# WangFeng18/3d-gaussian-splatting

Hardware: NVIDIA H100
Metric: render+backward FPS @1080p (2.4M Gaussians) (higher is better)
Workload: dtype f32

## Files before the change

### 3d-gaussian-splatting_b200/csrc/internal.h

```cpp
#pragma once
#include <cuda_runtime.h>
#include <stdint.h>

#include "../../include/gs_b200.h"
#include "project.cuh"

#define GS_GREC 12

struct GsFrameGeom {
  int width, height, wp, hp, ntx, nty, n_tiles;
  float fx, fy;
};

struct GsCrop {
  int left, top, width, height;
};

struct GsAuxOut {
  float bg[3];
  float* aux;
  float* aux_final;
};

#ifdef __CUDACC__
__device__ __forceinline__ void gs_store_aux(const GsAuxOut& ax, int ix, int iy, int wp, const GsCrop& crop,
                                             float depth, float alpha) {
  if (ax.aux) *reinterpret_cast<float2*>(ax.aux + ((size_t)iy * wp + ix) * 2) = make_float2(depth, alpha);
  const int x = ix - crop.left, y = iy - crop.top;
  if (ax.aux_final && x >= 0 && x < crop.width && y >= 0 && y < crop.height)
    *reinterpret_cast<float2*>(ax.aux_final + ((size_t)y * crop.width + x) * 2) = make_float2(depth, alpha);
}
template <int PX>
__device__ __forceinline__ void gs_load_aux_grad(const float* __restrict__ aux, const float* __restrict__ grad_aux,
                                                 int grad_is_final, int ix0, int iy, int wp, const GsCrop& crop,
                                                 float (&gD)[PX], float (&gA)[PX], float (&R)[PX]) {
#pragma unroll
  for (int p = 0; p < PX; ++p) {
    const size_t off = ((size_t)iy * wp + ix0 + p) * 2;
    const float2 da = *reinterpret_cast<const float2*>(aux + off);
    float2 g = make_float2(0.f, 0.f);
    if (!grad_is_final) {
      g = *reinterpret_cast<const float2*>(grad_aux + off);
    } else {
      const int x = ix0 + p - crop.left, y = iy - crop.top;
      if (x >= 0 && x < crop.width && y >= 0 && y < crop.height)
        g = *reinterpret_cast<const float2*>(grad_aux + ((size_t)y * crop.width + x) * 2);
    }
    gD[p] = g.x;
    gA[p] = g.y;
    R[p] = fmaf(g.x, da.x, fmaf(g.y, da.y, R[p]));
  }
}
#endif

struct GsRayPtrs {
  const float *rays_o, *lefttop, *dx, *dy;
};

struct GsTuning {
  int fwd_kernel;
  int fwd_ch;
  int bwd_kernel;
  int bwd_px;
  int bwd_ws;
  int bwd_unroll;
  int bwd_stages;
  int bwd_minb;
  int bwd_rq;
  int fwd_px;
  int bwd_ch;
  int strict;
  int gather;
  int sh_tc;
  int blend_repack;
};
GsTuning& gs_tuning();

void gs_count_launch(int n = 1);

int gs_sh_basis_count(int d);
int gs_sh_stream_width(int d);
int gs_sh_grad_width(int d);
int gs_sh_tc_mode(int d);
cudaError_t gs_launch_blend_sh_fwd(const float4* pA, const float2* pB, const float* pS, const GsRec* grec,
                                   const float* rgb, const uint32_t* ids, const uint32_t* goff , int d,
                                   const int* tile_accum,
                                   const GsFrameGeom& g, const GsRayPtrs& r, float* image, int* tile_neff,
                                   float* final_img, const GsCrop& crop, cudaStream_t st,
                                   const GsAuxOut* aux = nullptr );
cudaError_t gs_launch_blend_sh_bwd(const float4* pA, const float2* pB, const float* pS, const GsRec* grec,
                                   const float* rgb, const uint32_t* ids, const uint32_t* goff , int d,
                                   const int* tile_accum,
                                   const GsFrameGeom& g, const GsRayPtrs& r, const float* image,
                                   const float* grad_image, float* grad_inst, int grad_is_final, const GsCrop& crop,
                                   uint32_t* row_epoch, uint32_t epoch, int* tile_neff_b, cudaStream_t st,
                                   const float* aux = nullptr, const float* grad_aux = nullptr );

cudaError_t gs_launch_blend_sh_fwd_tc(const GsRec* grec, const float* rgb, const uint32_t* ids, int d,
                                      const int* tile_accum, const GsFrameGeom& g, const GsRayPtrs& r, float* image,
                                      int* tile_neff, float* final_img, const GsCrop& crop, cudaStream_t st,
                                      const GsAuxOut* aux = nullptr);
cudaError_t gs_launch_blend_sh_bwd_tc(const GsRec* grec, const float* rgb, const uint32_t* ids, const uint32_t* goff, int d,
                                      const int* tile_accum, const GsFrameGeom& g, const GsRayPtrs& r, const float* image,
                                      const float* grad_image, float* grad_inst, int grad_is_final, const GsCrop& crop,
                                      uint32_t* row_epoch, uint32_t epoch, int* tile_neff_b, cudaStream_t st,
                                      const float* aux = nullptr, const float* grad_aux = nullptr);

cudaError_t gs_launch_fused_project(const float* pos, const float* rgb, const float* opa, const float* quat,
                                    const float* scale, int n, int d, int scale_act, const GsCam& cam,
                                    const GsTileGrid& grid, float near_plane, float half_w, float half_h,
                                    GsRec* rec, uint2* rect ,
                                    uint32_t* count, uint32_t* dkey, int64_t* mask, unsigned int* n_visible, cudaStream_t st,
                                    bool sh_gaussian = false ,
                                    const GsFilter2d* filt = nullptr ,
                                    const float* f3d = nullptr ,
                                    const GsLens* lens = nullptr );

struct GsView {
  GsCam cam;
  GsTileGrid grid;
  GsFilter2d filt;
  float half_w, half_h, fx, fy;
};

cudaError_t gs_launch_fused_project_batch(const float* pos, const float* rgb, const float* opa, const float* quat,
                                          const float* scale, int n, int n_views, int d, int scale_act,
                                          const GsView* views, float near_plane, GsRec* rec ,
                                          uint2* rect , uint32_t* count , uint32_t* dkey ,
                                          int64_t* mask , unsigned int* n_visible,
                                          cudaStream_t st, bool sh_gaussian, bool filt,
                                          const float* f3d = nullptr ,
                                          const GsLens* lenses = nullptr );

struct GsGradPush {
  float* bucket;
// ... 167 lines not shown
```

### 3d-gaussian-splatting_b200/csrc/project.cu

```cuda
#include "internal.h"
#include "sh_common.cuh"

namespace {

constexpr int kBlock = 256;
constexpr float kInf = __builtin_huge_valf();

__global__ void __launch_bounds__(kBlock) jacobian_kernel(const float* __restrict__ pc, int n,
                                                           float* __restrict__ jac) {
  int i = blockIdx.x * kBlock + threadIdx.x;
  if (i >= n) return;
  float u0 = pc[3 * i], u1 = pc[3 * i + 1], u2 = pc[3 * i + 2];
  float rs = rsqrtf(u0 * u0 + u1 * u1 + u2 * u2);
  float* j = jac + 9 * (size_t)i;
  j[0] = 1.f / u2;
  j[1] = 0.f;
  j[2] = -u0 / (u2 * u2);
  j[3] = 0.f;
  j[4] = 1.f / u2;
  j[5] = -u1 / (u2 * u2);
  j[6] = rs * u0;
  j[7] = rs * u1;
  j[8] = rs * u2;
}


__device__ __forceinline__ void view_dir(const GsCam& cam, const float p[3], float dir[3], float& inv_len) {
  float u[3];
#pragma unroll
  for (int j = 0; j < 3; ++j) u[j] = p[j] + (cam.r[j] * cam.t[0] + cam.r[3 + j] * cam.t[1] + cam.r[6 + j] * cam.t[2]);
  inv_len = 1.f / sqrtf(u[0] * u[0] + u[1] * u[1] + u[2] * u[2]);
#pragma unroll
  for (int j = 0; j < 3; ++j) dir[j] = u[j] * inv_len;
}

template <int K>
__device__ __forceinline__ void sh_logits(const float* coef, const float* Y, float l[3]) {
#pragma unroll
  for (int c = 0; c < 3; ++c) {
    float s = 0.f;
#pragma unroll
    for (int k = 0; k < K; ++k) s = fmaf(Y[k], coef[c * K + k], s);
    l[c] = s;
  }
}

template <int KG, bool F = false, bool G3 = false, bool L = false>
__device__ __forceinline__ void fused_project_body(
    const float* __restrict__ pos, const float* __restrict__ rgb, const float* __restrict__ opa,
    const float* __restrict__ quat, const float* __restrict__ scale, int n, int d, int scale_act, const GsCam& cam,
    const GsTileGrid& grid, float near_plane, float half_w, float half_h, GsRec* __restrict__ rec,
    uint2* __restrict__ rect, uint32_t* __restrict__ count, uint32_t* __restrict__ dkey, int64_t* __restrict__ mask,
    unsigned int* __restrict__ n_visible, GsFilter2d filt = GsFilter2d{}, const float* __restrict__ f3d = nullptr,
    GsLens lens = GsLens{}) {
  static_assert(!G3 || F, "the 3-D filter runs in the 2-D filter's kernels");
  static_assert(!L || G3, "the lens runs in the 3-D filter's kernels");
  int i = blockIdx.x * kBlock + threadIdx.x;
  bool vis = false;
  uint32_t cnt = 0;
  if (i < n) {
    float p[3] = {pos[3 * i], pos[3 * i + 1], pos[3 * i + 2]};
    float q[4], s[3], raw_s[3], qn;
    gs_load_activated(quat, scale, i, scale_act, q, s, raw_s, qn);
    float f3 = 0.f, dl2o3 = 0.f;
    if constexpr (G3) {
      float s0[3];
      f3 = (L && !f3d) ? 0.f : f3d[i];
      gs_filter3d(f3, s, s0, dl2o3);
    }
    const float opa_raw = opa[i];
    float rgb_raw[3] = {0.f, 0.f, 0.f};
    if (KG == 0 && d == 3) {
      rgb_raw[0] = rgb[3 * i];
      rgb_raw[1] = rgb[3 * i + 1];
      rgb_raw[2] = rgb[3 * i + 2];
    }
    GsProj o = gs_project(cam, p, q, s, near_plane, L ? kInf : half_w, L ? kInf : half_h);
    if constexpr (L) {
      float J[4];
      gs_lens_project(lens, o, half_w, half_h, J);
    }
    vis = o.visible;
    if (mask) mask[i] = o.visible ? 1 : 0;
    bool keep = o.visible;
    float dl2o = 0.f;
    if constexpr (F) {
      const GsFilter2dOut fo = gs_filter2d(filt, o.a, o.b, o.c, o.d);
      o.a = fo.a;
      o.d = fo.d;
      dl2o = fo.dl2o;
      keep = keep && fo.keep;
    }
    uint2 rc = make_uint2(0u, 0u);
    if (keep) {
      uint32_t tx0, tx1, ty0, ty1;
      if (gs_tile_rect(grid, o.x, o.y, o.a, o.b, o.c, o.d, tx0, tx1, ty0, ty1)) {
        cnt = (tx1 - tx0) * (ty1 - ty0);
        rc = make_uint2(tx0 | (ty0 << 16), (tx1 - tx0) | ((ty1 - ty0) << 16));
        GsConic k = gs_make_conic(o.a, o.b, o.c, o.d);
        float op = gs_sigmoid(opa_raw);
        GsRec* r = rec + i;
        r->a = make_float4(o.x, o.y, k.ca, k.cb);
        float cr = 0.f, cg = 0.f, cb = 0.f;
        if constexpr (KG > 0) {
          float coef[3 * KG], dir[3], il, Y[KG], l[3];
#pragma unroll
          for (int k = 0; k < 3 * KG; ++k) coef[k] = rgb[(size_t)i * (3 * KG) + k];
          view_dir(cam, p, dir, il);
          gs_sh::sh_basis<KG>(dir[0], dir[1], dir[2], Y);
          sh_logits<KG>(coef, Y, l);
          cr = gs_sigmoid(l[0]);
          cg = gs_sigmoid(l[1]);
          cb = gs_sigmoid(l[2]);
        } else if (d == 3) {
          cr = gs_sigmoid(rgb_raw[0]);
          cg = gs_sigmoid(rgb_raw[1]);
          cb = gs_sigmoid(rgb_raw[2]);
        }
        float l2o = log2f(op);
        if constexpr (G3) {
          if (f3 != 0.f) l2o += dl2o3;
        }
        r->b = make_float4(k.cc, F ? l2o + dl2o : l2o, cr, cg);
        r->c = make_float4(cb, o.depth, __uint_as_float(rc.x), __uint_as_float(rc.y));
        r->d = make_uint4(0u, 0u, 0u, 0u);
      }
    }
    rect[i] = rc;
    count[i] = cnt;
    dkey[i] = cnt ? __float_as_uint(o.depth) : 0xffffffffu;
  }
  __shared__ unsigned long long wsum[kBlock / 32];
  unsigned long long c64 = cnt;
#pragma unroll
  for (int o = 16; o; o >>= 1) c64 += __shfl_xor_sync(0xffffffffu, c64, o);
  if ((threadIdx.x & 31) == 0) wsum[threadIdx.x >> 5] = c64;
  int nv = __syncthreads_count(vis);
  if (threadIdx.x == 0) {
    unsigned long long tot = 0;
#pragma unroll
    for (int w = 0; w < kBlock / 32; ++w) tot += wsum[w];
    if (nv) atomicAdd(n_visible, (unsigned int)nv);
    if (tot) atomicAdd(reinterpret_cast<unsigned long long*>(n_visible + 2), tot);
  }
}

__global__ void __launch_bounds__(kBlock) fused_project_kernel(
    const float* __restrict__ pos, const float* __restrict__ rgb, const float* __restrict__ opa,
    const float* __restrict__ quat, const float* __restrict__ scale, int n, int d, int scale_act, GsCam cam,
    GsTileGrid grid, float near_plane, float half_w, float half_h, GsRec* __restrict__ rec,
    uint2* __restrict__ rect, uint32_t* __restrict__ count, uint32_t* __restrict__ dkey, int64_t* __restrict__ mask,
    unsigned int* __restrict__ n_visible) {
  fused_project_body<0>(pos, rgb, opa, quat, scale, n, d, scale_act, cam, grid, near_plane, half_w, half_h, rec, rect,
                        count, dkey, mask, n_visible);
}

template <int K>
__global__ void __launch_bounds__(kBlock) fused_project_sh_kernel(
    const float* __restrict__ pos, const float* __restrict__ rgb, const float* __restrict__ opa,
    const float* __restrict__ quat, const float* __restrict__ scale, int n, int scale_act, GsCam cam,
    GsTileGrid grid, float near_plane, float half_w, float half_h, GsRec* __restrict__ rec,
    uint2* __restrict__ rect, uint32_t* __restrict__ count, uint32_t* __restrict__ dkey, int64_t* __restrict__ mask,
    unsigned int* __restrict__ n_visible) {
  fused_project_body<K>(pos, rgb, opa, quat, scale, n, 3 * K, scale_act, cam, grid, near_plane, half_w, half_h, rec,
                        rect, count, dkey, mask, n_visible);
}

template <int K>
__global__ void __launch_bounds__(kBlock) fused_project_filt_kernel(
    const float* __restrict__ pos, const float* __restrict__ rgb, const float* __restrict__ opa,
    const float* __restrict__ quat, const float* __restrict__ scale, int n, int d, int scale_act, GsCam cam,
    GsTileGrid grid, float near_plane, float half_w, float half_h, GsRec* __restrict__ rec,
    uint2* __restrict__ rect, uint32_t* __restrict__ count, uint32_t* __restrict__ dkey, int64_t* __restrict__ mask,
    unsigned int* __restrict__ n_visible, GsFilter2d filt) {
  fused_project_body<K, true>(pos, rgb, opa, quat, scale, n, d, scale_act, cam, grid, near_plane, half_w, half_h, rec,
                              rect, count, dkey, mask, n_visible, filt);
}

template <int K>
__global__ void __launch_bounds__(kBlock) fused_project_filt3_kernel(
    const float* __restrict__ pos, const float* __restrict__ rgb, const float* __restrict__ opa,
    const float* __restrict__ quat, const float* __restrict__ scale, int n, int d, int scale_act, GsCam cam,
    GsTileGrid grid, float near_plane, float half_w, float half_h, GsRec* __restrict__ rec,
    uint2* __restrict__ rect, uint32_t* __restrict__ count, uint32_t* __restrict__ dkey, int64_t* __restrict__ mask,
    unsigned int* __restrict__ n_visible, GsFilter2d filt, const float* __restrict__ f3d) {
  fused_project_body<K, true, true>(pos, rgb, opa, quat, scale, n, d, scale_act, cam, grid, near_plane, half_w, half_h,
                                    rec, rect, count, dkey, mask, n_visible, filt, f3d);
}

template <int K>
__global__ void __launch_bounds__(kBlock) fused_project_lens_kernel(
    const float* __restrict__ pos, const float* __restrict__ rgb, const float* __restrict__ opa,
    const float* __restrict__ quat, const float* __restrict__ scale, int n, int d, int scale_act, GsCam cam,
    GsTileGrid grid, float near_plane, float half_w, float half_h, GsRec* __restrict__ rec,
    uint2* __restrict__ rect, uint32_t* __restrict__ count, uint32_t* __restrict__ dkey, int64_t* __restrict__ mask,
    unsigned int* __restrict__ n_visible, GsFilter2d filt, const float* __restrict__ f3d, GsLens lens) {
  fused_project_body<K, true, true, true>(pos, rgb, opa, quat, scale, n, d, scale_act, cam, grid, near_plane, half_w,
                                          half_h, rec, rect, count, dkey, mask, n_visible, filt, f3d, lens);
}

template <int KG, bool F, bool G3 = false, bool L = false>
__device__ __forceinline__ uint32_t fused_project_one(
    const float* __restrict__ rgb, int i, int d, const GsCam& cam, const GsTileGrid& grid, float near_plane,
    float half_w, float half_h, const GsFilter2d& filt, const float p[3], const float q[4], const float s[3],
    float opa_raw, const float rgb_raw[3], uint32_t ty_off, int j, GsRec* __restrict__ rec, uint2* __restrict__ rect,
    uint32_t* __restrict__ count, uint32_t* __restrict__ dkey, int64_t* __restrict__ mask, bool& vis,
    float f3 = 0.f, float dl2o3 = 0.f, const GsLens* __restrict__ lens = nullptr) {
  uint32_t cnt = 0;
  {
    GsProj o = gs_project(cam, p, q, s, near_plane, L ? kInf : half_w, L ? kInf : half_h);
    if constexpr (L) {
      float J[4];
      gs_lens_project(*lens, o, half_w, half_h, J);
    }
    vis = o.visible;
    if (mask) mask[j] = o.visible ? 1 : 0;
    bool keep = o.visible;
    float dl2o = 0.f;
    if constexpr (F) {
      const GsFilter2dOut fo = gs_filter2d(filt, o.a, o.b, o.c, o.d);
      o.a = fo.a;
      o.d = fo.d;
      dl2o = fo.dl2o;
      keep = keep && fo.keep;
    }
    uint2 rc = make_uint2(0u, 0u);
    if (keep) {
      uint32_t tx0, tx1, ty0, ty1;
      if (gs_tile_rect(grid, o.x, o.y, o.a, o.b, o.c, o.d, tx0, tx1, ty0, ty1)) {
        cnt = (tx1 - tx0) * (ty1 - ty0);
        rc = make_uint2(tx0 | ((ty0 + ty_off) << 16), (tx1 - tx0) | ((ty1 - ty0) << 16));
        GsConic k = gs_make_conic(o.a, o.b, o.c, o.d);
        float op = gs_sigmoid(opa_raw);
        GsRec* r = rec + j;
        r->a = make_float4(o.x, o.y, k.ca, k.cb);
        float cr = 0.f, cg = 0.f, cb = 0.f;
        if constexpr (KG > 0) {
          float coef[3 * KG], dir[3], il, Y[KG], l[3];
#pragma unroll
          for (int k = 0; k < 3 * KG; ++k) coef[k] = rgb[(size_t)i * (3 * KG) + k];
          view_dir(cam, p, dir, il);
          gs_sh::sh_basis<KG>(dir[0], dir[1], dir[2], Y);
          sh_logits<KG>(coef, Y, l);
          cr = gs_sigmoid(l[0]);
          cg = gs_sigmoid(l[1]);
          cb = gs_sigmoid(l[2]);
        } else if (d == 3) {
          cr = gs_sigmoid(rgb_raw[0]);
          cg = gs_sigmoid(rgb_raw[1]);
          cb = gs_sigmoid(rgb_raw[2]);
        }
        float l2o = log2f(op);
        if constexpr (G3) {
          if (f3 != 0.f) l2o += dl2o3;
        }
        r->b = make_float4(k.cc, F ? l2o + dl2o : l2o, cr, cg);
        r->c = make_float4(cb, o.depth, __uint_as_float(rc.x), __uint_as_float(rc.y));
        r->d = make_uint4(0u, 0u, 0u, 0u);
      }
    }
    rect[j] = rc;
    count[j] = cnt;
    dkey[j] = cnt ? __float_as_uint(o.depth) : 0xffffffffu;
  }
  return cnt;
}

template <int K, bool F, bool G3, bool L = false>
__device__ __forceinline__ void fused_project_batch_body(
    const float* __restrict__ pos, const float* __restrict__ rgb, const float* __restrict__ opa,
    const float* __restrict__ quat, const float* __restrict__ scale, int n, int n_views, int d, int scale_act,
    const GsView* __restrict__ views, float near_plane, GsRec* __restrict__ rec, uint2* __restrict__ rect,
    uint32_t* __restrict__ count, uint32_t* __restrict__ dkey, int64_t* __restrict__ mask,
    unsigned int* __restrict__ n_visible, const float* __restrict__ f3d, const GsLens* __restrict__ lenses = nullptr) {
  const int i = blockIdx.x * kBlock + threadIdx.x;
  unsigned int nv = 0;
  unsigned long long c64 = 0;
  if (i < n) {
    float p[3] = {pos[3 * i], pos[3 * i + 1], pos[3 * i + 2]};
    float q[4], s[3], raw_s[3], qn;
    gs_load_activated(quat, scale, i, scale_act, q, s, raw_s, qn);
    float f3 = 0.f, dl2o3 = 0.f;
    if constexpr (G3) {
      float s0[3];
      f3 = (L && !f3d) ? 0.f : f3d[i];
      gs_filter3d(f3, s, s0, dl2o3);
    }
    const float opa_raw = opa[i];
    float rgb_raw[3] = {0.f, 0.f, 0.f};
    if (K == 0 && d == 3) {
      rgb_raw[0] = rgb[3 * i];
      rgb_raw[1] = rgb[3 * i + 1];
      rgb_raw[2] = rgb[3 * i + 2];
    }
    for (int v = 0; v < n_views; ++v) {
      const GsView vw = views[v];
      bool vis = false;
      c64 += fused_project_one<K, F, G3, L>(rgb, i, d, vw.cam, vw.grid, near_plane, vw.half_w, vw.half_h, vw.filt, p,
                                            q, s, opa_raw, rgb_raw, (uint32_t)(v * vw.grid.nty), v * n + i, rec, rect,
                                            count, dkey, mask, vis, f3, dl2o3, lenses + v);
      nv += vis ? 1u : 0u;
    }
  }
  __shared__ unsigned long long wsum[kBlock / 32];
  __shared__ unsigned int wvis[kBlock / 32];
#pragma unroll
  for (int o = 16; o; o >>= 1) {
    c64 += __shfl_xor_sync(0xffffffffu, c64, o);
    nv += __shfl_xor_sync(0xffffffffu, nv, o);
  }
  if ((threadIdx.x & 31) == 0) {
    wsum[threadIdx.x >> 5] = c64;
    wvis[threadIdx.x >> 5] = nv;
  }
  __syncthreads();
  if (threadIdx.x == 0) {
    unsigned long long tot = 0;
    unsigned int tv = 0;
#pragma unroll
    for (int w = 0; w < kBlock / 32; ++w) {
      tot += wsum[w];
      tv += wvis[w];
    }
    if (tv) atomicAdd(n_visible, tv);
    if (tot) atomicAdd(reinterpret_cast<unsigned long long*>(n_visible + 2), tot);
  }
}

#define GS_PBATCH_PARAMS                                                                                            \
  const float* __restrict__ pos, const float* __restrict__ rgb, const float* __restrict__ opa,                     \
      const float* __restrict__ quat, const float* __restrict__ scale, int n, int n_views, int d, int scale_act,   \
      const GsView* __restrict__ views, float near_plane, GsRec* __restrict__ rec, uint2* __restrict__ rect,        \
      uint32_t* __restrict__ count, uint32_t* __restrict__ dkey, int64_t* __restrict__ mask,                        \
      unsigned int* __restrict__ n_visible
#define GS_PBATCH_ARGS \
  pos, rgb, opa, quat, scale, n, n_views, d, scale_act, views, near_plane, rec, rect, count, dkey, mask, n_visible

template <int K, bool F>
__global__ void __launch_bounds__(kBlock) fused_project_batch_kernel(GS_PBATCH_PARAMS) {
  fused_project_batch_body<K, F, false>(GS_PBATCH_ARGS, nullptr);
}

template <int K>
__global__ void __launch_bounds__(kBlock) fused_project_batch_filt3_kernel(GS_PBATCH_PARAMS,
                                                                           const float* __restrict__ f3d) {
  fused_project_batch_body<K, true, true>(GS_PBATCH_ARGS, f3d);
}

template <int K>
__global__ void __launch_bounds__(kBlock) fused_project_batch_lens_kernel(GS_PBATCH_PARAMS,
                                                                          const float* __restrict__ f3d,
                                                                          const GsLens* __restrict__ lenses) {
  fused_project_batch_body<K, true, true, true>(GS_PBATCH_ARGS, f3d, lenses);
}
#undef GS_PBATCH_PARAMS

template <int W>
__device__ __forceinline__ float* push_dst(const GsGradPush& P, float* local, int cnt) {
  if (W == 0) return local;
  const uint32_t idx = (uint32_t)(local - P.bucket);
  const uint32_t owner = idx / P.per;
  if (cnt > 1 && (idx + (uint32_t)cnt - 1) / P.per != owner) return nullptr;
  if (owner == (uint32_t)P.rank) return local;
  float* st = P.staging[0];
#pragma unroll
  for (int p = 1; p < (W > 0 ? W : 1); ++p)
    if (owner == (uint32_t)p) st = P.staging[p];
  return st + (size_t)P.rank * P.per + (idx - owner * P.per);
}

template <int W, int CNT>
__device__ __forceinline__ void push_store(const GsGradPush& P, float* local, const float* v) {
  float* dst = push_dst<W>(P, local, CNT);
  if (dst) {
#pragma unroll
    for (int k = 0; k < CNT; ++k) dst[k] = v[k];
  } else {
#pragma unroll
    for (int k = 0; k < CNT; ++k) *push_dst<W>(P, local + k, 1) = v[k];
  }
}

template <int D, int GW, int W, bool DT, int KG, bool CG = false, bool F = false, bool G3 = false, bool L = false>
__device__ __forceinline__ void fused_project_bwd_body(
    const float* __restrict__ pos, const float* __restrict__ rgb, const float* __restrict__ opa,
    const float* __restrict__ quat, const float* __restrict__ scale, int n, int scale_act, GsCam cam,
    float near_plane, float half_w, float half_h, const uint32_t* __restrict__ offsets_g,
    const uint32_t* __restrict__ count, const float* __restrict__ grad_inst,
    const uint32_t* __restrict__ row_epoch, uint32_t epoch, float* __restrict__ g_pos,
    float* __restrict__ g_rgb, float* __restrict__ g_opa, float* __restrict__ g_quat, float* __restrict__ g_scale,
    GsGradPush push, float* cg = nullptr, GsFilter2d filt = GsFilter2d{}, const float* __restrict__ f3d = nullptr,
    GsLens lens = GsLens{}) {
  static_assert(KG == 0 || (D == 3 * KG && GW == GS_GREC), "per-Gaussian SH: 3K coefficients, RGB gradient rows");
  static_assert(!G3 || F, "the 3-D filter runs in the 2-D filter's kernels");
  static_assert(!L || (G3 && W == 0), "the lens runs in the 3-D filter's kernels, without a push");
  static_assert(!CG || (W == 0 && GW == GS_GREC), "camera gradient: RGB gradient rows, no push");
  constexpr int DC = KG ? 3 : D;
  int i = blockIdx.x * kBlock + threadIdx.x;
  constexpr bool kStagedRgb = (D != 3) && (W == 0);
  const bool valid = i < n;
  if (!valid && !kStagedRgb) return;
  float gp[3] = {0.f, 0.f, 0.f}, gq_raw[4] = {0.f, 0.f, 0.f, 0.f}, gs_raw[3] = {0.f, 0.f, 0.f};
  float go = 0.f;
  float acc[GW];
#pragma unroll
  for (int k = 0; k < GW; ++k) acc[k] = 0.f;
  float gsh[KG ? D : 1];
#pragma unroll
// ... 1204 lines not shown
```

### 3d-gaussian-splatting_b200/csrc/render.cu

```cuda
#include <cub/device/device_radix_sort.cuh>
#include <cub/device/device_scan.cuh>
#include <cub/iterator/counting_input_iterator.cuh>
#include <cub/iterator/transform_input_iterator.cuh>

#include <cmath>
#include <cstdio>
#include <cstdlib>
#include <cstring>
#include <new>

#include "internal.h"

struct GsCountInSortedOrder {
  const uint32_t* count;
  const uint32_t* perm;
  uint32_t n;
  __host__ __device__ __forceinline__ uint32_t operator()(uint32_t i) const { return i < n ? count[perm[i]] : 0u; }
};

static thread_local char g_err[512] = {0};

int gs_set_error(cudaError_t e, const char* what) {
  snprintf(g_err, sizeof(g_err), "CUDA error %d (%s) at %s", (int)e, cudaGetErrorString(e), what);
  return (int)e;
// ... 340 lines not shown
    const double c[5] = {1.0, 3.0 * l.k[0], 5.0 * l.k[1], 7.0 * l.k[2], 9.0 * l.k[3]};
    const double half_pi = 1.5707963267948966;
    const double t = first_nonpositive(c, 4, half_pi * half_pi);
    if (!(t < half_pi * half_pi)) return INFINITY;
    const double r = tan(sqrt(t));
    return r * r;
  }
  return INFINITY;
}

static bool lens_is_centre_pinhole(const gs_lens& l, const gs_camera& cam) {
  return l.model == GS_LENS_PINHOLE && (double)l.cx == cam.width / 2.0 && (double)l.cy == cam.height / 2.0;
}

static GsLens lens_constants(const gs_lens& l, const gs_camera& cam) {
  GsLens L{};
  L.model = l.model;
  L.ox = (float)(((double)l.cx - cam.width / 2.0) / (double)cam.focal_x);
  L.oy = (float)(((double)l.cy - cam.height / 2.0) / (double)cam.focal_y);
  L.rho2_max = (float)lens_rho2_max(l);
  if (l.model != GS_LENS_PINHOLE)
    for (int k = 0; k < 4; ++k) L.k[k] = l.k[k];
  return L;
}

static int resolve_lenses(const gs_ctx* c, const gs_camera* cams, int n_views, GsLens* out, bool& on, const char* who) {
  on = false;
  if (c->lens_n == 0) return 0;
  if (c->lens_n != 1 && c->lens_n != n_views)
    return gs_fail(GS_ERR_INVALID_ARG, who, "the context's lenses are set for another number of views (n must be 1 or B)");
  for (int v = 0; v < n_views; ++v) {
    const gs_lens& l = c->lens_set[c->lens_n == 1 ? 0 : v];
    if (!lens_is_centre_pinhole(l, cams[v])) on = true;
    out[v] = lens_constants(l, cams[v]);
  }
  return 0;
}

static GsView view_constants(const gs_ctx* c, const gs_camera* cam, const GsFrameGeom& g) {
  GsView v{};
  if (c->filter2d != GS_FILTER2D_NONE) {
    v.filt.ex = (float)((double)c->filter2d_var / ((double)cam->focal_x * (double)cam->focal_x));
    v.filt.ey = (float)((double)c->filter2d_var / ((double)cam->focal_y * (double)cam->focal_y));
    v.filt.compensate = c->filter2d == GS_FILTER2D_ANTIALIAS;
  }
  v.grid.lx = (float)(16.0 / (double)cam->focal_x);
  v.grid.ly = (float)(16.0 / (double)cam->focal_y);
  v.grid.leftmost = (float)(-(double)g.wp / 2.0 / (double)cam->focal_x);
  v.grid.topmost = (float)(-(double)g.hp / 2.0 / (double)cam->focal_y);
  v.grid.t2 = -2.f * logf(cam->tile_thresh);
  v.grid.ntx = g.wp / GS_TILE;
  v.grid.nty = g.hp / GS_TILE;
  memcpy(v.cam.r, cam->rot, sizeof(v.cam.r));
  memcpy(v.cam.t, cam->tran, sizeof(v.cam.t));
  v.half_w = (float)((double)cam->width * 1.2 / 2.0 / (double)cam->focal_x);
  v.half_h = (float)((double)cam->height * 1.2 / 2.0 / (double)cam->focal_y);
  v.fx = cam->focal_x;
  v.fy = cam->focal_y;
  return v;
}

static int reserve_frame(gs_ctx* c, size_t N, int n_tiles, cudaStream_t st) {
  GS_CUDA_TRY(c->rec.reserve(N * sizeof(GsRec), st));
  GS_CUDA_TRY(c->rect.reserve(N * sizeof(uint2), st));
  GS_CUDA_TRY(c->count.reserve((N + 1) * 4, st));
  GS_CUDA_TRY(c->offsets.reserve((N + 1) * 4, st));
  GS_CUDA_TRY(c->dkey_in.reserve(N * 4 + 4, st));
  GS_CUDA_TRY(c->dkey_out.reserve(N * 4 + 4, st));
  GS_CUDA_TRY(c->perm.reserve(N * 4 + 4, st));
  GS_CUDA_TRY(c->offsets_g.reserve((N + 1) * 4, st));
  GS_CUDA_TRY(c->tile_accum.reserve((size_t)(n_tiles + 1) * 4, st));
  GS_CUDA_TRY(c->tile_neff.reserve((size_t)n_tiles * 4, st));
  GS_CUDA_TRY(c->tile_neff_b.reserve((size_t)n_tiles * 4, st));
  GS_CUDA_TRY(c->counters.reserve(64, st));
  if (c->iota_n < N) {
    GS_CUDA_TRY(c->iota.reserve(N * 4 + 4, st));
    GS_CUDA_TRY(gs_launch_iota(c->iota.as<uint32_t>(), (int)N, st));
    gs_count_launch();
    c->iota_n = N;
  }
  return 0;
}

static int bin_frame(gs_ctx* c, int n, const GsFrameGeom& g, bool gather, int blend_d, int d, const float* rgb,
                     cudaStream_t st, long long& m_out) {
  gs_mark(c, 1, st);
  size_t tmp_bytes = 0, tmp2 = 0, tmp3 = 0;
  if (n > 0)
    GS_CUDA_TRY(cub::DeviceRadixSort::SortPairs(nullptr, tmp_bytes, c->dkey_in.as<uint32_t>(),
                                                c->dkey_out.as<uint32_t>(), c->iota.as<uint32_t>(),
                                                c->perm.as<uint32_t>(), n, 0, 32, st));
  GsCountInSortedOrder cnt_it_fn{c->count.as<uint32_t>(), c->perm.as<uint32_t>(), (uint32_t)n};
  cub::CountingInputIterator<uint32_t> idx_it(0);
  cub::TransformInputIterator<uint32_t, GsCountInSortedOrder, cub::CountingInputIterator<uint32_t>> cnt_it(idx_it,
                                                                                                            cnt_it_fn);
  GS_CUDA_TRY(cub::DeviceScan::ExclusiveSum(nullptr, tmp2, cnt_it, c->offsets.as<uint32_t>(), n + 1, st));
  GS_CUDA_TRY(cub::DeviceScan::ExclusiveSum(nullptr, tmp3, c->count.as<uint32_t>(), c->offsets_g.as<uint32_t>(),
                                            n + 1, st));
  if (tmp2 > tmp_bytes) tmp_bytes = tmp2;
  if (tmp3 > tmp_bytes) tmp_bytes = tmp3;
  GS_CUDA_TRY(c->cub_tmp.reserve(tmp_bytes, st));
  GS_CUDA_TRY(cub::DeviceScan::ExclusiveSum(c->cub_tmp.p, tmp3, c->count.as<uint32_t>(), c->offsets_g.as<uint32_t>(),
                                            n + 1, st));
  *c->host_m = 0;
  GS_CUDA_TRY(cudaMemcpyAsync(c->host_m, c->counters.as<unsigned int>() + 2, 8, cudaMemcpyDeviceToHost, st));
  GS_CUDA_TRY(cudaEventRecord(c->ev_m, st));
  if (n > 0)
    GS_CUDA_TRY(cub::DeviceRadixSort::SortPairs(c->cub_tmp.p, tmp_bytes, c->dkey_in.as<uint32_t>(),
                                                c->dkey_out.as<uint32_t>(), c->iota.as<uint32_t>(),
                                                c->perm.as<uint32_t>(), n, 0, 32, st));
  GS_CUDA_TRY(cub::DeviceScan::ExclusiveSum(c->cub_tmp.p, tmp2, cnt_it, c->offsets.as<uint32_t>(), n + 1, st));
  GS_CUDA_TRY(cudaEventSynchronize(c->ev_m));
  if (*c->host_m >= (1ull << 31))
    return gs_set_error_msg(GS_ERR_UNSUPPORTED, "gs_render_forward: more than 2^31 tile instances");
  const long long m = (long long)*c->host_m;
  const size_t M = (size_t)m;
  m_out = m;

  gs_mark(c, 2, st);
  static const int forced_key = getenv("GS_TILE_KEY_BYTES") ? atoi(getenv("GS_TILE_KEY_BYTES")) : 0;
  const int key_bytes = (g.n_tiles <= 65536 && forced_key != 4) ? 2 : 4;
  const size_t crow = blend_d == 3 ? 16 : (size_t)gs_sh_stream_width(d) * 4;
  if (!gather) {
    GS_CUDA_TRY(c->pA.reserve(M * 16 + 16, st));
    GS_CUDA_TRY(c->pC.reserve(M * crow + 16, st));
    GS_CUDA_TRY(c->pB.reserve((M + 2) * 8, st));
  }
  if (m > 0) {
    GS_CUDA_TRY(c->keys_in.reserve(M * 4 + 16, st));
    GS_CUDA_TRY(c->keys_out.reserve(M * 4 + 16, st));
    GS_CUDA_TRY(c->vals_in.reserve(M * 4, st));
    GS_CUDA_TRY(c->vals_out.reserve(M * 4, st));
    GS_CUDA_TRY(gs_launch_emit_keys(c->rect.as<uint2>(), c->perm.as<uint32_t>(), c->offsets.as<uint32_t>(), n, g.ntx,
                                    c->keys_in.p, key_bytes, c->vals_in.as<uint32_t>(), st));
    gs_count_launch();
    gs_mark(c, 3, st);
    int end_bit = ceil_log2((unsigned)g.n_tiles);
    if (end_bit < 1) end_bit = 1;
    size_t sort_tmp = 0;
    if (key_bytes == 2) {
      GS_CUDA_TRY(cub::DeviceRadixSort::SortPairs(nullptr, sort_tmp, c->keys_in.as<uint16_t>(),
                                                  c->keys_out.as<uint16_t>(), c->vals_in.as<uint32_t>(),
                                                  c->vals_out.as<uint32_t>(), (int)m, 0, end_bit, st));
      GS_CUDA_TRY(c->cub_tmp.reserve(sort_tmp, st));
      GS_CUDA_TRY(cub::DeviceRadixSort::SortPairs(c->cub_tmp.p, sort_tmp, c->keys_in.as<uint16_t>(),
                                                  c->keys_out.as<uint16_t>(), c->vals_in.as<uint32_t>(),
                                                  c->vals_out.as<uint32_t>(), (int)m, 0, end_bit, st));
    } else {
      GS_CUDA_TRY(cub::DeviceRadixSort::SortPairs(nullptr, sort_tmp, c->keys_in.as<uint32_t>(),
                                                  c->keys_out.as<uint32_t>(), c->vals_in.as<uint32_t>(),
                                                  c->vals_out.as<uint32_t>(), (int)m, 0, end_bit, st));
      GS_CUDA_TRY(c->cub_tmp.reserve(sort_tmp, st));
      GS_CUDA_TRY(cub::DeviceRadixSort::SortPairs(c->cub_tmp.p, sort_tmp, c->keys_in.as<uint32_t>(),
                                                  c->keys_out.as<uint32_t>(), c->vals_in.as<uint32_t>(),
                                                  c->vals_out.as<uint32_t>(), (int)m, 0, end_bit, st));
    }
  }
  if (m == 0) gs_mark(c, 3, st);
  gs_mark(c, 4, st);
  if (gather) {
    GS_CUDA_TRY(gs_launch_tile_ranges(c->keys_out.p, key_bytes, m, g.n_tiles, c->tile_accum.as<int>(), st));
  } else if (blend_d == 3) {
    GS_CUDA_TRY(gs_launch_pack_sorted(c->keys_out.p, key_bytes, c->vals_out.as<uint32_t>(), m, g.n_tiles, g.ntx,
                                      c->rec.as<GsRec>(), c->offsets_g.as<uint32_t>(), c->pA.as<float4>(),
                                      c->pB.as<float2>(), c->pC.as<float4>(), c->tile_accum.as<int>(), st));
  } else {
    GS_CUDA_TRY(gs_launch_pack_sorted_sh(c->keys_out.p, key_bytes, c->vals_out.as<uint32_t>(), m, g.n_tiles, g.ntx,
                                         c->rec.as<GsRec>(), c->offsets_g.as<uint32_t>(), rgb, d,
                                         gs_sh_stream_width(d), c->pA.as<float4>(), c->pB.as<float2>(),
                                         c->pC.as<float>(), c->tile_accum.as<int>(), st));
  }
  if (m > 0) gs_count_launch();
  return 0;
}

static int render_forward_impl(gs_ctx* c, const char* who, const float* pos, const float* rgb, const float* opa,
                               const float* quat, const float* scale, int n, int d, int scale_activation,
                               const gs_camera* cam, float* image, float* final_img, int64_t* culling_mask,
                               gs_stream_t stream, const gs_render_aux* ax = nullptr,
                               const gs_render_feat* ft = nullptr) {
  if (!c || !cam || n < 0) return gs_fail(GS_ERR_INVALID_ARG, who, "bad arguments");
  if (d != 3 && gs_sh_basis_count(d) == 0)
    return gs_fail(GS_ERR_UNSUPPORTED, who, "colour width must be 3 (RGB), 27 (SH deg 2) or 48 (SH deg 3)");
  if (int rc = check_camera(*cam, who)) return rc;
  if (!image || (n > 0 && (!pos || !rgb || !opa || !quat || !scale)))
    return gs_fail(GS_ERR_INVALID_ARG, who, "null tensor pointer");
  const bool sh_gaussian = d != 3 && c->sh_eval == GS_SH_EVAL_GAUSSIAN;
  const int blend_d = sh_gaussian ? 3 : d;
  const bool filt_on = c->filter2d != GS_FILTER2D_NONE;
  GsAuxOut aux_out;
  bool use_aux;
  if (int rc = parse_aux(ax, final_img, aux_out, use_aux, who)) return rc;
  if (use_aux)
    if (int rc = gs_blend_aux_supported(blend_d, true, ax->aux != nullptr)) return rc;
  const bool gather = gs_tuning().gather != 0;
  if (ft) {
    if (!gs_feat_width_ok(ft->f)) return gs_fail(GS_ERR_INVALID_ARG, who, "f must be 8, 16 or 32");
// ... 927 lines not shown
```

### 3d-gaussian-splatting_b200/csrc/surfel.cu

```cuda
#include "internal.h"
#include "sh_common.cuh"

namespace {

constexpr int kBlock = 256;

__device__ __forceinline__ void surfel_view_dir(const GsCam& cam, const float p[3], float dir[3], float& inv_len) {
  float u[3];
#pragma unroll
  for (int j = 0; j < 3; ++j) u[j] = p[j] + (cam.r[j] * cam.t[0] + cam.r[3 + j] * cam.t[1] + cam.r[6 + j] * cam.t[2]);
  inv_len = 1.f / sqrtf(u[0] * u[0] + u[1] * u[1] + u[2] * u[2]);
#pragma unroll
  for (int j = 0; j < 3; ++j) dir[j] = u[j] * inv_len;
}

template <int K>
__device__ __forceinline__ void surfel_sh_logits(const float* coef, const float* Y, float l[3]) {
#pragma unroll
  for (int c = 0; c < 3; ++c) {
    float s = 0.f;
#pragma unroll
    for (int k = 0; k < K; ++k) s = fmaf(Y[k], coef[c * K + k], s);
    l[c] = s;
  }
}

__device__ __forceinline__ void cam_rot(const GsCam& cam, const float v[3], float o[3]) {
#pragma unroll
  for (int r = 0; r < 3; ++r) o[r] = cam.r[3 * r] * v[0] + cam.r[3 * r + 1] * v[1] + cam.r[3 * r + 2] * v[2];
}
__device__ __forceinline__ void cam_rot_t(const GsCam& cam, const float v[3], float o[3]) {
#pragma unroll
  for (int k = 0; k < 3; ++k) o[k] = cam.r[k] * v[0] + cam.r[3 + k] * v[1] + cam.r[6 + k] * v[2];
}

struct SurfelGeom {
  float u[3], v[3], nc[3], pc[3];
  float Rr0[3], Rr1[3];
  GsRot Q;
};
__device__ __forceinline__ SurfelGeom surfel_geom(const GsCam& cam, const float p[3], const float q[4], const float s[3]) {
  SurfelGeom g;
  g.Q = gs_quat_to_rot(q[0], q[1], q[2], q[3]);
  const float r0[3] = {g.Q.m[0], g.Q.m[3], g.Q.m[6]};
  const float r1[3] = {g.Q.m[1], g.Q.m[4], g.Q.m[7]};
  const float r2[3] = {g.Q.m[2], g.Q.m[5], g.Q.m[8]};
  cam_rot(cam, r0, g.Rr0);
  cam_rot(cam, r1, g.Rr1);
  cam_rot(cam, r2, g.nc);
  gs_world_to_cam(cam, p, g.pc);
#pragma unroll
  for (int k = 0; k < 3; ++k) {
    g.u[k] = s[0] * g.Rr0[k];
    g.v[k] = s[1] * g.Rr1[k];
  }
  return g;
}

__device__ __forceinline__ bool surfel_tile_rect(const GsTileGrid& g, float left, float right, float top, float bottom,
                                                 uint32_t& tx0, uint32_t& tx1, uint32_t& ty0, uint32_t& ty1) {
  ty0 = (uint32_t)fmaxf((top - g.topmost) / g.ly, 0.f);
  ty1 = (uint32_t)((bottom - g.topmost) / g.ly + 1.f);
  tx0 = (uint32_t)fmaxf((left - g.leftmost) / g.lx, 0.f);
  tx1 = (uint32_t)((right - g.leftmost) / g.lx + 1.f);
  ty1 = min(ty1, (uint32_t)g.nty);
  tx1 = min(tx1, (uint32_t)g.ntx);
  return (ty1 > ty0) && (tx1 > tx0);
}

template <int KG>
__global__ void __launch_bounds__(kBlock) surfel_project_kernel(
    const float* __restrict__ pos, const float* __restrict__ rgb, const float* __restrict__ opa,
    const float* __restrict__ quat, const float* __restrict__ scale, int n, int scale_act, GsCam cam, GsTileGrid grid,
    float near_plane, float half_w, float half_h, float fx, float fy, GsSurfelRec* __restrict__ rec,
    uint2* __restrict__ rect, uint32_t* __restrict__ count, uint32_t* __restrict__ dkey, int64_t* __restrict__ mask,
    unsigned int* __restrict__ n_visible) {
  const int i = blockIdx.x * kBlock + threadIdx.x;
  bool vis = false;
  uint32_t cnt = 0;
  if (i < n) {
    const float p[3] = {pos[3 * i], pos[3 * i + 1], pos[3 * i + 2]};
    float q[4], s[3], raw_s[3], qn;
    gs_load_activated(quat, scale, i, scale_act, q, s, raw_s, qn);
    const SurfelGeom G = surfel_geom(cam, p, q, s);
    float zc = G.pc[2];
    if (zc > near_plane) {
      const float cx = G.pc[0] / zc, cy = G.pc[1] / zc;
      vis = fabsf(cx) < half_w && fabsf(cy) < half_h;
    }
    if (mask) mask[i] = vis ? 1 : 0;
    uint2 rc = make_uint2(0u, 0u);
    if (vis) {
      const float c22 = 9.f * (G.u[2] * G.u[2] + G.v[2] * G.v[2]) - G.pc[2] * G.pc[2];
      if (c22 < 0.f) {
        const float c00 = 9.f * (G.u[0] * G.u[0] + G.v[0] * G.v[0]) - G.pc[0] * G.pc[0];
        const float c11 = 9.f * (G.u[1] * G.u[1] + G.v[1] * G.v[1]) - G.pc[1] * G.pc[1];
        const float c02 = 9.f * (G.u[0] * G.u[2] + G.v[0] * G.v[2]) - G.pc[0] * G.pc[2];
        const float c12 = 9.f * (G.u[1] * G.u[2] + G.v[1] * G.v[2]) - G.pc[1] * G.pc[2];
        const float ex = c02 / c22, ey = c12 / c22;
        const float hx = sqrtf(fmaxf(ex * ex - c00 / c22, 0.f));
        const float hy = sqrtf(fmaxf(ey * ey - c11 / c22, 0.f));
        const float cx = G.pc[0] / G.pc[2], cy = G.pc[1] / G.pc[2];
        const float rx = 0.70710678f / fx, ry = 0.70710678f / fy;
        const float left = fminf(ex - hx, cx - rx), right = fmaxf(ex + hx, cx + rx);
        const float top = fminf(ey - hy, cy - ry), bottom = fmaxf(ey + hy, cy + ry);
        uint32_t tx0, tx1, ty0, ty1;
        if (surfel_tile_rect(grid, left, right, top, bottom, tx0, tx1, ty0, ty1)) {
          cnt = (tx1 - tx0) * (ty1 - ty0);
          rc = make_uint2(tx0 | (ty0 << 16), (tx1 - tx0) | ((ty1 - ty0) << 16));
          GsSurfelRec r;
#pragma unroll
          for (int k = 0; k < 3; ++k) {
            r.M[3 * k] = G.u[k];
            r.M[3 * k + 1] = G.v[k];
            r.M[3 * k + 2] = G.pc[k];
          }
          r.op = gs_sigmoid(opa[i]);
          if constexpr (KG > 0) {
            float coef[3 * KG], dir[3], il, Y[KG], l[3];
#pragma unroll
            for (int k = 0; k < 3 * KG; ++k) coef[k] = rgb[(size_t)i * (3 * KG) + k];
            surfel_view_dir(cam, p, dir, il);
            gs_sh::sh_basis<KG>(dir[0], dir[1], dir[2], Y);
            surfel_sh_logits<KG>(coef, Y, l);
#pragma unroll
            for (int c = 0; c < 3; ++c) r.rgb[c] = gs_sigmoid(l[c]);
          } else {
#pragma unroll
            for (int c = 0; c < 3; ++c) r.rgb[c] = gs_sigmoid(rgb[3 * i + c]);
          }
          const float sgn = (G.nc[0] * G.pc[0] + G.nc[1] * G.pc[1] + G.nc[2] * G.pc[2]) > 0.f ? -1.f : 1.f;
#pragma unroll
          for (int k = 0; k < 3; ++k) r.nrm[k] = sgn * G.nc[k];
          float4* dst = reinterpret_cast<float4*>(rec + i);
          const float4* src = reinterpret_cast<const float4*>(&r);
#pragma unroll
          for (int k = 0; k < 4; ++k) dst[k] = src[k];
        }
      }
    }
    rect[i] = rc;
    count[i] = cnt;
    dkey[i] = cnt ? __float_as_uint(zc) : 0xffffffffu;
  }
  __shared__ unsigned long long wsum[kBlock / 32];
  unsigned long long c64 = cnt;
#pragma unroll
  for (int o = 16; o; o >>= 1) c64 += __shfl_xor_sync(0xffffffffu, c64, o);
  if ((threadIdx.x & 31) == 0) wsum[threadIdx.x >> 5] = c64;
  const int nv = __syncthreads_count(vis);
  if (threadIdx.x == 0) {
    unsigned long long tot = 0;
#pragma unroll
    for (int w = 0; w < kBlock / 32; ++w) tot += wsum[w];
    if (nv) atomicAdd(n_visible, (unsigned int)nv);
    if (tot) atomicAdd(reinterpret_cast<unsigned long long*>(n_visible + 2), tot);
  }
}

template <int KG>
__global__ void __launch_bounds__(kBlock) surfel_project_bwd_kernel(
    const float* __restrict__ pos, const float* __restrict__ rgb, const float* __restrict__ opa,
    const float* __restrict__ quat, const float* __restrict__ scale, int n, int scale_act, GsCam cam,
    const uint32_t* __restrict__ offsets_g, const uint32_t* __restrict__ count, const float* __restrict__ grad_inst,
    const uint32_t* __restrict__ row_epoch, uint32_t epoch, float* __restrict__ g_pos, float* __restrict__ g_rgb,
    float* __restrict__ g_opa, float* __restrict__ g_quat, float* __restrict__ g_scale) {
  constexpr int D = KG ? 3 * KG : 3;
  constexpr int GW = GS_SURFEL_GREC;
  const int i = blockIdx.x * kBlock + threadIdx.x;
  if (i >= n) return;
  float acc[GW];
#pragma unroll
  for (int k = 0; k < GW; ++k) acc[k] = 0.f;
  float gp[3] = {0.f, 0.f, 0.f}, gq_raw[4] = {0.f, 0.f, 0.f, 0.f}, gs_raw[3] = {0.f, 0.f, 0.f}, go = 0.f;
  float gcol[D];
#pragma unroll
  for (int k = 0; k < D; ++k) gcol[k] = 0.f;
  const uint32_t cnt = count[i], o0 = offsets_g[i];
  if (cnt > 0) {
    for (uint32_t r = o0; r < o0 + cnt; ++r) {
      if (row_epoch[r] != epoch) continue;
      const float4* row = reinterpret_cast<const float4*>(grad_inst + (size_t)r * GW);
#pragma unroll
      for (int qq = 0; qq < GW / 4; ++qq) {
        const float4 v = row[qq];
        acc[4 * qq] += v.x;
        acc[4 * qq + 1] += v.y;
        acc[4 * qq + 2] += v.z;
        acc[4 * qq + 3] += v.w;
      }
    }
    const float p[3] = {pos[3 * i], pos[3 * i + 1], pos[3 * i + 2]};
    float q[4], s[3], raw_s[3], qn;
    gs_load_activated(quat, scale, i, scale_act, q, s, raw_s, qn);
    const SurfelGeom G = surfel_geom(cam, p, q, s);
    float gu[3], gv[3], gpc[3], gn[3];
#pragma unroll
    for (int k = 0; k < 3; ++k) {
      gu[k] = acc[3 * k];
      gv[k] = acc[3 * k + 1];
      gpc[k] = acc[3 * k + 2];
      gn[k] = acc[13 + k];
    }
    const float sgn = (G.nc[0] * G.pc[0] + G.nc[1] * G.pc[1] + G.nc[2] * G.pc[2]) > 0.f ? -1.f : 1.f;
    float gsv[3];
    gsv[0] = gu[0] * G.Rr0[0] + gu[1] * G.Rr0[1] + gu[2] * G.Rr0[2];
    gsv[1] = gv[0] * G.Rr1[0] + gv[1] * G.Rr1[1] + gv[2] * G.Rr1[2];
    gsv[2] = 0.f;
    float gr0[3], gr1[3], gr2[3];
    cam_rot_t(cam, gu, gr0);
    cam_rot_t(cam, gv, gr1);
    cam_rot_t(cam, gn, gr2);
    cam_rot_t(cam, gpc, gp);
    float gR[9];
#pragma unroll
    for (int k = 0; k < 3; ++k) {
      gR[3 * k] = s[0] * gr0[k];
      gR[3 * k + 1] = s[1] * gr1[k];
      gR[3 * k + 2] = sgn * gr2[k];
    }
    const float w = q[0], x = q[1], y = q[2], z = q[3];
    float gq[4];
    gq[0] = 2.f * (-z * gR[1] + y * gR[2] + z * gR[3] - x * gR[5] - y * gR[6] + x * gR[7]);
    gq[1] = 2.f * (y * gR[1] + z * gR[2] + y * gR[3] - 2.f * x * gR[4] - w * gR[5] + z * gR[6] + w * gR[7] - 2.f * x * gR[8]);
    gq[2] = 2.f * (-2.f * y * gR[0] + x * gR[1] + w * gR[2] + x * gR[3] + z * gR[5] - w * gR[6] + z * gR[7] - 2.f * y * gR[8]);
    gq[3] = 2.f * (-2.f * z * gR[0] - w * gR[1] + x * gR[2] + w * gR[3] - 2.f * z * gR[4] + y * gR[5] + x * gR[6] + y * gR[7]);
    const float dot = q[0] * gq[0] + q[1] * gq[1] + q[2] * gq[2] + q[3] * gq[3];
#pragma unroll
    for (int k = 0; k < 4; ++k) gq_raw[k] = (gq[k] - q[k] * dot) / qn;
#pragma unroll
    for (int k = 0; k < 2; ++k) {
      if (scale_act == GS_SCALE_ABS)
        gs_raw[k] = gsv[k] * (raw_s[k] > 0.f ? 1.f : (raw_s[k] < 0.f ? -1.f : 0.f));
      else
        gs_raw[k] = gsv[k] * expf(fminf(fmaxf(raw_s[k], -1.f), 1.f));
    }
    const float op = gs_sigmoid(opa[i]);
    go = acc[9] * op * (1.f - op);
    if constexpr (KG > 0) {
// ... 84 lines not shown
```

Baseline: 489.4.

## Track depth key range in projection and shrink depth radix sort bits

Projection kernels now compute a block-reduced min and max of visible depth keys and publish them with atomicMax into the counters buffer. The host reads them back before the depth sort and restricts the radix sort to only the bit range that varies, so fewer passes run. To get the range in time, the host synchronisation is moved before the sort, which takes away the overlap with the first scan and adds a host stall. Keys for non-visible entries (0xffffffff) still need to sort last, so the bit-count computation extends the range until kmax's low bits are all ones. It also assumes counters 4 and 5 are zeroed each frame.

```diff
diff --git a/3d-gaussian-splatting_b200/csrc/internal.h b/3d-gaussian-splatting_b200/csrc/internal.h
--- a/3d-gaussian-splatting_b200/csrc/internal.h
+++ b/3d-gaussian-splatting_b200/csrc/internal.h
@@ -51,6 +51,26 @@
     R[p] = fmaf(g.x, da.x, fmaf(g.y, da.y, R[p]));
   }
 }
+__device__ __forceinline__ void gs_dkey_range_warp(uint32_t kinv, uint32_t kmax, uint32_t* s_inv, uint32_t* s_max) {
+  kinv = __reduce_max_sync(0xffffffffu, kinv);
+  kmax = __reduce_max_sync(0xffffffffu, kmax);
+  if ((threadIdx.x & 31) == 0) {
+    s_inv[threadIdx.x >> 5] = kinv;
+    s_max[threadIdx.x >> 5] = kmax;
+  }
+}
+__device__ __forceinline__ void gs_dkey_range_flush(const uint32_t* s_inv, const uint32_t* s_max, int warps,
+                                                    unsigned int* counters) {
+  uint32_t kinv = 0, kmax = 0;
+  for (int w = 0; w < warps; ++w) {
+    kinv = max(kinv, s_inv[w]);
+    kmax = max(kmax, s_max[w]);
+  }
+  if (kinv | kmax) {
+    atomicMax(counters + 4, kinv);
+    atomicMax(counters + 5, kmax);
+  }
+}
 #endif
 
 struct GsRayPtrs {
diff --git a/3d-gaussian-splatting_b200/csrc/project.cu b/3d-gaussian-splatting_b200/csrc/project.cu
--- a/3d-gaussian-splatting_b200/csrc/project.cu
+++ b/3d-gaussian-splatting_b200/csrc/project.cu
@@ -57,7 +57,7 @@
   static_assert(!L || G3, "the lens runs in the 3-D filter's kernels");
   int i = blockIdx.x * kBlock + threadIdx.x;
   bool vis = false;
-  uint32_t cnt = 0;
+  uint32_t cnt = 0, kinv = 0, kmax = 0;
   if (i < n) {
     float p[3] = {pos[3 * i], pos[3 * i + 1], pos[3 * i + 2]};
     float q[4], s[3], raw_s[3], qn;
@@ -129,12 +129,18 @@
     rect[i] = rc;
     count[i] = cnt;
     dkey[i] = cnt ? __float_as_uint(o.depth) : 0xffffffffu;
+    if (cnt && __float_as_uint(o.depth) != 0xffffffffu) {
+      kinv = ~__float_as_uint(o.depth);
+      kmax = __float_as_uint(o.depth);
+    }
   }
   __shared__ unsigned long long wsum[kBlock / 32];
+  __shared__ uint32_t wkinv[kBlock / 32], wkmax[kBlock / 32];
   unsigned long long c64 = cnt;
 #pragma unroll
   for (int o = 16; o; o >>= 1) c64 += __shfl_xor_sync(0xffffffffu, c64, o);
   if ((threadIdx.x & 31) == 0) wsum[threadIdx.x >> 5] = c64;
+  gs_dkey_range_warp(kinv, kmax, wkinv, wkmax);
   int nv = __syncthreads_count(vis);
   if (threadIdx.x == 0) {
     unsigned long long tot = 0;
@@ -142,6 +148,7 @@
     for (int w = 0; w < kBlock / 32; ++w) tot += wsum[w];
     if (nv) atomicAdd(n_visible, (unsigned int)nv);
     if (tot) atomicAdd(reinterpret_cast<unsigned long long*>(n_visible + 2), tot);
+    gs_dkey_range_flush(wkinv, wkmax, kBlock / 32, n_visible);
   }
 }
 
@@ -205,7 +212,7 @@
     float half_w, float half_h, const GsFilter2d& filt, const float p[3], const float q[4], const float s[3],
     float opa_raw, const float rgb_raw[3], uint32_t ty_off, int j, GsRec* __restrict__ rec, uint2* __restrict__ rect,
     uint32_t* __restrict__ count, uint32_t* __restrict__ dkey, int64_t* __restrict__ mask, bool& vis,
-    float f3 = 0.f, float dl2o3 = 0.f, const GsLens* __restrict__ lens = nullptr) {
+    uint32_t& kinv, uint32_t& kmax, float f3 = 0.f, float dl2o3 = 0.f, const GsLens* __restrict__ lens = nullptr) {
   uint32_t cnt = 0;
   {
     GsProj o = gs_project(cam, p, q, s, near_plane, L ? kInf : half_w, L ? kInf : half_h);
@@ -262,6 +269,10 @@
     rect[j] = rc;
     count[j] = cnt;
     dkey[j] = cnt ? __float_as_uint(o.depth) : 0xffffffffu;
+    if (cnt && __float_as_uint(o.depth) != 0xffffffffu) {
+      kinv = max(kinv, ~__float_as_uint(o.depth));
+      kmax = max(kmax, __float_as_uint(o.depth));
+    }
   }
   return cnt;
 }
@@ -276,6 +287,7 @@
   const int i = blockIdx.x * kBlock + threadIdx.x;
   unsigned int nv = 0;
   unsigned long long c64 = 0;
+  uint32_t kinv = 0, kmax = 0;
   if (i < n) {
     float p[3] = {pos[3 * i], pos[3 * i + 1], pos[3 * i + 2]};
     float q[4], s[3], raw_s[3], qn;
@@ -298,12 +310,15 @@
       bool vis = false;
       c64 += fused_project_one<K, F, G3, L>(rgb, i, d, vw.cam, vw.grid, near_plane, vw.half_w, vw.half_h, vw.filt, p,
                                             q, s, opa_raw, rgb_raw, (uint32_t)(v * vw.grid.nty), v * n + i, rec, rect,
-                                            count, dkey, mask, vis, f3, dl2o3, lenses + v);
+                                            count, dkey, mask, vis, kinv, kmax, f3, dl2o3,
+                                            lenses + v);
       nv += vis ? 1u : 0u;
     }
   }
   __shared__ unsigned long long wsum[kBlock / 32];
   __shared__ unsigned int wvis[kBlock / 32];
+  __shared__ uint32_t wkinv[kBlock / 32], wkmax[kBlock / 32];
+  gs_dkey_range_warp(kinv, kmax, wkinv, wkmax);
 #pragma unroll
   for (int o = 16; o; o >>= 1) {
     c64 += __shfl_xor_sync(0xffffffffu, c64, o);
@@ -324,6 +339,7 @@
     }
     if (tv) atomicAdd(n_visible, tv);
     if (tot) atomicAdd(reinterpret_cast<unsigned long long*>(n_visible + 2), tot);
+    gs_dkey_range_flush(wkinv, wkmax, kBlock / 32, n_visible);
   }
 }
 
diff --git a/3d-gaussian-splatting_b200/csrc/render.cu b/3d-gaussian-splatting_b200/csrc/render.cu
--- a/3d-gaussian-splatting_b200/csrc/render.cu
+++ b/3d-gaussian-splatting_b200/csrc/render.cu
@@ -446,6 +446,14 @@
   return 0;
 }
 
+static int depth_sort_bits(uint32_t kinv, uint32_t kmax) {
+  const uint32_t kmin = ~kinv;
+  if (kmin > kmax) return 1;
+  int e = kmin == kmax ? 0 : 32 - __builtin_clz(kmin ^ kmax);
+  while (e < 32 && (kmax & ((1u << e) - 1u)) == (1u << e) - 1u) ++e;
+  return e < 1 ? 1 : e;
+}
+
 static int bin_frame(gs_ctx* c, int n, const GsFrameGeom& g, bool gather, int blend_d, int d, const float* rgb,
                      cudaStream_t st, long long& m_out) {
   gs_mark(c, 1, st);
@@ -464,19 +472,21 @@
   if (tmp2 > tmp_bytes) tmp_bytes = tmp2;
   if (tmp3 > tmp_bytes) tmp_bytes = tmp3;
   GS_CUDA_TRY(c->cub_tmp.reserve(tmp_bytes, st));
+  c->host_m[0] = c->host_m[1] = 0;
+  GS_CUDA_TRY(cudaMemcpyAsync(c->host_m, c->counters.as<unsigned int>() + 2, 16, cudaMemcpyDeviceToHost, st));
+  GS_CUDA_TRY(cudaEventRecord(c->ev_m, st));
   GS_CUDA_TRY(cub::DeviceScan::ExclusiveSum(c->cub_tmp.p, tmp3, c->count.as<uint32_t>(), c->offsets_g.as<uint32_t>(),
                                             n + 1, st));
-  *c->host_m = 0;
-  GS_CUDA_TRY(cudaMemcpyAsync(c->host_m, c->counters.as<unsigned int>() + 2, 8, cudaMemcpyDeviceToHost, st));
-  GS_CUDA_TRY(cudaEventRecord(c->ev_m, st));
-  if (n > 0)
+  GS_CUDA_TRY(cudaEventSynchronize(c->ev_m));
+  if (c->host_m[0] >= (1ull << 31))
+    return gs_set_error_msg(GS_ERR_UNSUPPORTED, "gs_render_forward: more than 2^31 tile instances");
+  if (n > 0) {
+    const uint32_t kinv = (uint32_t)c->host_m[1], kmax = (uint32_t)(c->host_m[1] >> 32);
     GS_CUDA_TRY(cub::DeviceRadixSort::SortPairs(c->cub_tmp.p, tmp_bytes, c->dkey_in.as<uint32_t>(),
                                                 c->dkey_out.as<uint32_t>(), c->iota.as<uint32_t>(),
-                                                c->perm.as<uint32_t>(), n, 0, 32, st));
+                                                c->perm.as<uint32_t>(), n, 0, depth_sort_bits(kinv, kmax), st));
+  }
   GS_CUDA_TRY(cub::DeviceScan::ExclusiveSum(c->cub_tmp.p, tmp2, cnt_it, c->offsets.as<uint32_t>(), n + 1, st));
-  GS_CUDA_TRY(cudaEventSynchronize(c->ev_m));
-  if (*c->host_m >= (1ull << 31))
-    return gs_set_error_msg(GS_ERR_UNSUPPORTED, "gs_render_forward: more than 2^31 tile instances");
   const long long m = (long long)*c->host_m;
   const size_t M = (size_t)m;
   m_out = m;
diff --git a/3d-gaussian-splatting_b200/csrc/surfel.cu b/3d-gaussian-splatting_b200/csrc/surfel.cu
--- a/3d-gaussian-splatting_b200/csrc/surfel.cu
+++ b/3d-gaussian-splatting_b200/csrc/surfel.cu
@@ -77,7 +77,7 @@
     unsigned int* __restrict__ n_visible) {
   const int i = blockIdx.x * kBlock + threadIdx.x;
   bool vis = false;
-  uint32_t cnt = 0;
+  uint32_t cnt = 0, kinv = 0, kmax = 0;
   if (i < n) {
     const float p[3] = {pos[3 * i], pos[3 * i + 1], pos[3 * i + 2]};
     float q[4], s[3], raw_s[3], qn;
@@ -142,12 +142,18 @@
     rect[i] = rc;
     count[i] = cnt;
     dkey[i] = cnt ? __float_as_uint(zc) : 0xffffffffu;
+    if (cnt && __float_as_uint(zc) != 0xffffffffu) {
+      kinv = ~__float_as_uint(zc);
+      kmax = __float_as_uint(zc);
+    }
   }
   __shared__ unsigned long long wsum[kBlock / 32];
+  __shared__ uint32_t wkinv[kBlock / 32], wkmax[kBlock / 32];
   unsigned long long c64 = cnt;
 #pragma unroll
   for (int o = 16; o; o >>= 1) c64 += __shfl_xor_sync(0xffffffffu, c64, o);
   if ((threadIdx.x & 31) == 0) wsum[threadIdx.x >> 5] = c64;
+  gs_dkey_range_warp(kinv, kmax, wkinv, wkmax);
   const int nv = __syncthreads_count(vis);
   if (threadIdx.x == 0) {
     unsigned long long tot = 0;
@@ -155,6 +161,7 @@
     for (int w = 0; w < kBlock / 32; ++w) tot += wsum[w];
     if (nv) atomicAdd(n_visible, (unsigned int)nv);
     if (tot) atomicAdd(reinterpret_cast<unsigned long long*>(n_visible + 2), tot);
+    gs_dkey_range_flush(wkinv, wkmax, kBlock / 32, n_visible);
   }
 }
 
```

New measurement: 495.8, median of 6. Within noise of the previous version (+1.3%).
